# PinataFarms/DAD-3DHeads

Measured on AMD Instinct MI355X. Metric: images/sec (FLAME decode + 445-lmk projection), batch 64 @ 256^2, higher is better.
Workload: dtype f32

## Files before the change

dad-3dheads_amd/_lib.py:

```python
from __future__ import annotations

import ctypes as C
import os

_HERE = os.path.dirname(os.path.abspath(__file__))
LIB_PATH = os.environ.get("DAD3D_LIB_PATH") or os.path.join(_HERE, "libdad3d_hip.so")

OK, E_INVALID, E_HIP, E_UNSUPPORTED, E_NOMEM = range(5)
ZERO_ROTATION, TO_2D, MUTATE_PARAMS, FLIP_Z, COMPAT_CROSS_B3 = 0x1, 0x2, 0x4, 0x8, 0x10
NORMAL_ACCUMULATE = 0x1
TEX_INDEX_CORNER, TEX_INDEX_REFERENCE = 0, 1
DTYPE_F32, DTYPE_U8 = 0, 1
EVAL_SELF_EXCLUDE, EVAL_MAX_K, EVAL_MAX_HEAD, EVAL_MAX_ANCHORS = 0x1, 8, 4096, 8
HEATMAP_RAW, HEATMAP_UINT8, HEATMAP_FLOAT = 0, 1, 2
OBJ_MAX_LINE_BYTES, OBJ_FLAG_NONFINITE, OBJ_FLAG_LARGE = 71, 0x1, 0x2
JSON_MAX_NUMBER_BYTES, JSON_MAX_LITERAL_BYTES, JSON_FLAG_NONFINITE = 23, 64, 0x1
JSON_PARSE_TILE_BYTES, JSON_PARSE_RECORD_INTS = 4096, 6
(JSON_PARSE_FLAG_GRAMMAR, JSON_PARSE_FLAG_DIGITS, JSON_PARSE_FLAG_BIG_INT, JSON_PARSE_FLAG_SUBNORMAL, JSON_PARSE_FLAG_OVERFLOW,
 JSON_PARSE_FLAG_AMBIGUOUS) = 0x1, 0x2, 0x4, 0x8, 0x10, 0x20
KERNEL_AUTO, KERNEL_TWO_ROLE, KERNEL_PIPELINED, KERNEL_SPLIT_BF16, KERNEL_SPLIT_F16 = 0, 1, 2, 3, 4


class Dad3dError(RuntimeError):
    def __init__(self, status: int, message: str):
        super().__init__(f"libdad3d_hip status {status}: {message}")
        self.status = status


class UnsupportedError(Dad3dError):
    pass


class FlameModelC(C.Structure):
    _fields_ = [
        ("n_verts", C.c_int32),
        ("n_betas", C.c_int32),
        ("n_joints", C.c_int32),
        ("v_template", C.c_void_p),
        ("shapedirs", C.c_void_p),
        ("posedirs", C.c_void_p),
        ("j_regressor", C.c_void_p),
        ("parents", C.c_void_p),
        ("lbs_weights", C.c_void_p),
    ]


class FlameConstsC(C.Structure):
    _fields_ = [(k, C.c_int32) for k in ("shape", "expression", "jaw", "rotation", "eyeballs", "neck", "translation", "scale")]


class LightC(C.Structure):
    _fields_ = [
        ("intensity_ambient", C.c_float),
# ... 122 lines not shown
```

dad-3dheads_amd/csrc/capi.cpp:

```cpp
#include <algorithm>
#include <cmath>
#include <cstdlib>
#include <cstring>
#include <memory>
#include <mutex>

#include "common.hpp"

namespace dad3d {

static thread_local std::string g_last_error;

void set_error(const char* fmt, ...) {
    char buf[1024];
    va_list ap;
    va_start(ap, fmt);
    vsnprintf(buf, sizeof buf, fmt, ap);
    va_end(ap);
    g_last_error = buf;
}

template <typename T>
static dad3d_status upload(T** dst, const std::vector<T>& src) {
    *dst = nullptr;
// ... 54 lines not shown
    int kernel_choice = -1;
    float* d_bwd_partials = nullptr;
    int bwd_cap = 0;
    float* d_grad_partials = nullptr;
    size_t grad_cap = 0;
    float* d_imgc = nullptr;
    unsigned* d_sync = nullptr;
    unsigned arrive_total = 0;
    int cap_nbb = 0;
    bool profiling = false;
    unsigned long long* d_trace = nullptr;
    uint64_t trace_capacity = 0;
    char* d_split_a = nullptr;
    int split_cap = 0;
    std::vector<char*> split_retired;
    hipEvent_t ev_first = nullptr, ev_last = nullptr;
    int prof_launches = 0;
    ~dad3d_flame() {
        DeviceGuard guard(device);
        for (void* p : {(void*)d_sync, (void*)d_imgc, (void*)d_bwd_partials, (void*)d_grad_partials, (void*)d_split_a}) (void)hipFree(p);
        for (char* p : split_retired) (void)hipFree(p);
        if (ev_first) (void)hipEventDestroy(ev_first);
        if (ev_last) (void)hipEventDestroy(ev_last);
    }
};

static int decode_kernel_choice() {
    static const int choice = [] {
        const char* e = getenv("DAD3D_DECODE_KERNEL");
        if (!e) return 0;
        if (e[0] == 'v' && e[1] == '1') return DAD3D_KERNEL_TWO_ROLE;
        if (std::strcmp(e, "split") == 0) return DAD3D_KERNEL_SPLIT_BF16;
        if (std::strcmp(e, "split_f16") == 0) return DAD3D_KERNEL_SPLIT_F16;
        return std::strcmp(e, "force_pipe") == 0 ? DAD3D_KERNEL_PIPELINED : DAD3D_KERNEL_AUTO;
    }();
    return choice;
}

static size_t frag_offset(int tile, int kgroups, int g, int col, int q) {
    return ((((size_t)tile * kgroups + g) * 4 + col / 16) * 64 + (col % 16) + 16 * q) * 4;
}
template <typename F>
static void for_each_fragment(std::vector<float>& pack, int n_tiles, int kgroups, F&& f) {
    for (int t = 0; t < n_tiles; ++t)
        for (int g = 0; g < kgroups; ++g)
            for (int col = 0; col < kTileCols; ++col)
                for (int q = 0; q < 4; ++q) f(t, g, col, q, &pack[frag_offset(t, kgroups, g, col, q)]);
}

static int grad_chunks(const dad3d_flame* h) { return (h->n_verts * 3 + kGradChunk - 1) / kGradChunk; }

static dad3d_status grad_inputs_prepare(dad3d_flame* h, int batch, hipStream_t s) {
    const int pad = (batch + kBlockImages - 1) / kBlockImages * kBlockImages;
    const int per_slice = grad_chunks_per_slice(pad);
    const size_t rows = (size_t)((grad_chunks(h) + per_slice - 1) / per_slice) * pad;
    bool need_pack;
    {
        std::lock_guard<std::mutex> lock(h->c->gpack_mutex);
        need_pack = h->c->d_gpack == nullptr;
    }
    const bool need_scratch = rows > h->grad_cap;
    if (!need_pack && !need_scratch) return DAD3D_OK;
    hipStreamCaptureStatus capture = hipStreamCaptureStatusNone;
    if (s != nullptr) (void)hipStreamIsCapturing(s, &capture);
    DAD3D_REQUIRE(capture == hipStreamCaptureStatusNone,
                  "the first training step of a handle (and the first at a larger batch) allocates: run it once before capturing a graph");
// ... 312 lines not shown
    if (s != nullptr) (void)hipStreamIsCapturing(s, &capture);
    DAD3D_REQUIRE(capture == hipStreamCaptureStatusNone, "the first fp16-split decode of a model builds its basis planes: run it once before capturing a graph");
    const size_t bytes = (size_t)c->n_tiles_pipe * kPipeKGroups * 4 * 64 * 4 * sizeof(float);
    float* d = nullptr;
    DAD3D_HIP_TRY(hipMalloc(reinterpret_cast<void**>(&d), bytes));
    dad3d_status st = launch_split_basis_f16(c->d_bpack_pipe, d, c->n_tiles_pipe, c->split_b_scale, s);
    if (st == DAD3D_OK && hipStreamSynchronize(s) != hipSuccess) {
        set_error("ensure_basis_f16: hipStreamSynchronize failed");
        st = DAD3D_E_HIP;
    }
    if (st) {
        (void)hipFree(d);
        return st;
    }
    c->d_bpack_f16 = d;
    return DAD3D_OK;
}

static dad3d_status ensure_split_scratch(dad3d_flame* h, int n_phase, hipStream_t s) {
    if (n_phase <= h->split_cap) return DAD3D_OK;
    hipStreamCaptureStatus capture = hipStreamCaptureStatusNone;
    if (s != nullptr) (void)hipStreamIsCapturing(s, &capture);
    DAD3D_REQUIRE(capture == hipStreamCaptureStatusNone,
                  "the first split-kernel decode of a handle (and the first at a larger batch) allocates: run it once before capturing a graph");
    if (h->d_split_a) h->split_retired.push_back(h->d_split_a);
    h->d_split_a = nullptr, h->split_cap = 0;
    DAD3D_HIP_TRY(hipMalloc(reinterpret_cast<void**>(&h->d_split_a), (size_t)n_phase * kSplitBlockBytes));
    DAD3D_HIP_TRY(hipMemsetAsync(h->d_split_a, 0, (size_t)n_phase * kSplitBlockBytes, s));
    h->split_cap = n_phase;
    return DAD3D_OK;
}

static int resolve_kernel(const dad3d_flame* h, int pinned, int batch, unsigned flags, bool posed) {
    const bool pipe_covers = h->c->d_bpack_pipe && !posed && !(flags & (DAD3D_COMPAT_CROSS_B3 | DAD3D_ZERO_ROTATION)) &&
                             (size_t)batch * h->n_verts * 12 < ((size_t)1 << 31) && (size_t)batch * std::max(h->lmk->n, 1) * 8 < ((size_t)1 << 31);
    if (pinned == DAD3D_KERNEL_TWO_ROLE || (pinned == DAD3D_KERNEL_AUTO && !pipe_covers)) return DAD3D_KERNEL_TWO_ROLE;
    if (pipe_covers) return pinned == DAD3D_KERNEL_AUTO ? DAD3D_KERNEL_PIPELINED : pinned;
    set_error("dad3d_flame_decode: the %s kernel does not cover this launch (model, flags or output size)",
              pinned == DAD3D_KERNEL_PIPELINED ? "pipelined" : "split");
    return -1;
}

static dad3d_status decode_impl(dad3d_flame* h, float* params, int batch, unsigned flags, float* verts3d, float* proj,
                                float* lmk_xy, int32_t* lmk_px, float* posed, void* stream) {
    DAD3D_REQUIRE(h, "dad3d_flame_decode: null handle");
    DAD3D_REQUIRE(batch >= 0, "dad3d_flame_decode: negative batch");
    if (batch == 0) return DAD3D_OK;
    DAD3D_REQUIRE(params, "dad3d_flame_decode: null params");
    DAD3D_REQUIRE(!((flags & DAD3D_FLIP_Z) && (flags & DAD3D_TO_2D)), "DAD3D_FLIP_Z needs a 3-component projection");
    DAD3D_REQUIRE(!(posed && (flags & DAD3D_COMPAT_CROSS_B3)), "DAD3D_COMPAT_CROSS_B3 is inference-only (dad3d_flame_decode_posed refuses it)");
    DeviceGuard guard(h->device);
    hipStream_t s = static_cast<hipStream_t>(stream);
    const int pinned = h->kernel_choice >= 0 ? h->kernel_choice : decode_kernel_choice();
    const int kernel = resolve_kernel(h, pinned, batch, flags, posed != nullptr);
    if (kernel < 0) return DAD3D_E_UNSUPPORTED;
    const LandmarkList& L = *h->lmk;
    const int n_lmk = (lmk_xy || lmk_px) ? L.n : 0;

    const bool on_sub = L.sub && !verts3d && !proj && n_lmk && !h->d_trace && pinned != DAD3D_KERNEL_PIPELINED;
    FlameConsts* c = on_sub ? L.sub.get() : h->c.get();
    const float4* vtab = on_sub ? L.d_sub_vtab : L.d_vtab;
    const int n_verts = on_sub ? L.sub_verts : h->n_verts;

    dad3d_status st;
    if (kernel == DAD3D_KERNEL_SPLIT_BF16 || kernel == DAD3D_KERNEL_SPLIT_F16) {
        DAD3D_REQUIRE(!h->d_trace, "dad3d_flame_decode: the split kernels have no trace stamps");
// ... 17 lines not shown
        sa.n_params = h->lay.n_params;
        sa.batch = batch;
        sa.n_phase = n_phase;
        sa.n_tiles = c->n_tiles_pipe;
        split_chunking(sa.n_tiles, n_phase, &sa.n_chunks, &sa.phases_per_chunk);
        sa.n_verts = n_verts;
        sa.n_lmk = n_lmk;
        sa.image_size = h->image_size;
        sa.flags = flags & 0xFFu;
        st = launch_flame_decode_split(sa, kernel, s);
    } else if (kernel == DAD3D_KERNEL_PIPELINED) {
        DAD3D_REQUIRE(!h->d_trace || h->trace_capacity >= trace_entries_pipe(h), "dad3d_flame_decode: the trace buffer holds %llu entries, "
                      "this launch stamps %llu (dad3d_flame_debug_trace_entries)", (unsigned long long)h->trace_capacity,
                      (unsigned long long)trace_entries_pipe(h));
        PipeArgs pa{};
        pa.params = params;
        pa.bpack = c->d_bpack_pipe;
        pa.vtab = vtab;
        pa.lmk_next = L.d_next;
        pa.verts3d = verts3d;
        pa.proj = proj;
        pa.lmk_xy = lmk_xy;
        pa.lmk_px = lmk_px;
        pa.trace = h->d_trace;
        pa.n_params = h->lay.n_params;
        pa.batch = batch;
        pa.n_half = (batch + kPipeHalf - 1) / kPipeHalf;
        pa.n_tiles = c->n_tiles_pipe;
        pa.n_verts = n_verts;
        pa.n_lmk = n_lmk;
        pa.image_size = h->image_size;
        pa.flags = flags & 0xFFu;
        pa.n_chunks = 1;
        if (!h->d_trace && (!proj || (flags & DAD3D_TO_2D))) pipe_chunking(pa.n_tiles, pa.n_half, &pa.chunk_half, &pa.n_chunks, &pa.wg_per_xcd);
        st = launch_flame_decode_pipe(pa, s);
    } else {
        DAD3D_REQUIRE(!h->d_trace || h->trace_capacity >= trace_entries_two_role(h, batch), "dad3d_flame_decode: the trace buffer holds %llu "
                      "entries, this launch stamps %llu (dad3d_flame_debug_trace_entries)", (unsigned long long)h->trace_capacity,
                      (unsigned long long)trace_entries_two_role(h, batch));
        if (posed && batch <= DAD3D_GRAD_INPUTS_MAX_BATCH && h->n_betas + 36 <= kGradRows && (st = grad_inputs_prepare(h, batch, s))) return st;
        const int nbb = (batch + kBlockImages - 1) / kBlockImages;
        if (nbb > h->cap_nbb) {
            DAD3D_HIP_TRY(hipDeviceSynchronize());
            if ((st = flame_reserve(h, nbb))) return st;
        }
        DecodeArgs da{};
        da.params = params;
        da.bpack = h->c->d_bpack;
        da.jdirs = h->c->d_jdirs;
        da.j0 = h->c->d_j0;
        da.weights8 = h->c->d_w8;
        da.lmk_head = L.d_head;
        da.lmk_next = L.d_next;
        da.imgc = h->d_imgc;
        da.sync = h->d_sync;
        da.verts3d = verts3d;
        da.proj = proj;
        da.lmk_xy = lmk_xy;
        da.lmk_px = lmk_px;
        da.posed = posed;
        da.trace = h->d_trace;
        da.lay = h->lay;
        std::copy(h->parents, h->parents + kNumJoints, da.parents);
        da.batch = batch;
        da.nbb = nbb;
        da.n_tiles = h->n_tiles;
// ... 51 lines not shown
    float* d_p = n_p ? d_par + n_par + n_v : nullptr;
    float* d_lx = n_lx ? d_par + n_par + n_v + n_p : nullptr;
    int32_t* d_lp = n_lp ? reinterpret_cast<int32_t*>(d_par + n_par + n_v + n_p + n_lx) : nullptr;
    dad3d_status st = DAD3D_OK;
    auto fail = [&](hipError_t e, const char* what) {
        if (e != hipSuccess && st == DAD3D_OK) {
            set_error("%s failed: %s", what, hipGetErrorString(e));
            st = DAD3D_E_HIP;
        }
    };
    fail(hipMemcpy(d_par, params, n_par * sizeof(float), hipMemcpyHostToDevice), "hipMemcpy(params)");
    if (!st) st = dad3d_flame_decode(h, d_par, batch, flags, d_v, d_p, d_lx, d_lp, nullptr);
    if (!st) fail(hipDeviceSynchronize(), "hipDeviceSynchronize");
    if (!st && (flags & DAD3D_MUTATE_PARAMS)) fail(hipMemcpy(params, d_par, n_par * sizeof(float), hipMemcpyDeviceToHost), "hipMemcpy");
    if (!st && n_v) fail(hipMemcpy(verts3d, d_v, n_v * sizeof(float), hipMemcpyDeviceToHost), "hipMemcpy");
    if (!st && n_p) fail(hipMemcpy(proj, d_p, n_p * sizeof(float), hipMemcpyDeviceToHost), "hipMemcpy");
    if (!st && n_lx) fail(hipMemcpy(lmk_xy, d_lx, n_lx * sizeof(float), hipMemcpyDeviceToHost), "hipMemcpy");
    if (!st && n_lp) fail(hipMemcpy(lmk_px, d_lp, n_lp * sizeof(int32_t), hipMemcpyDeviceToHost), "hipMemcpy");
    (void)hipFree(d);
    return st;
}

dad3d_status dad3d_flame_readjust_params(dad3d_flame* h, float* params, int batch, const float* pads_scale,
                                         float pad_left, float pad_top, float scale, void* stream) {
    DAD3D_REQUIRE(h && batch >= 0, "dad3d_flame_readjust_params: bad argument");
    if (batch == 0) return DAD3D_OK;
    DAD3D_REQUIRE(params, "dad3d_flame_readjust_params: null params");
    DeviceGuard guard(h->device);
    return launch_readjust(params, batch, h->lay, pads_scale, pad_left, pad_top, scale, h->image_size,
                           static_cast<hipStream_t>(stream));
}

dad3d_status dad3d_flame_select_kernel(dad3d_flame* h, int which) {
    DAD3D_REQUIRE(h && which >= DAD3D_KERNEL_AUTO && which <= DAD3D_KERNEL_SPLIT_F16, "dad3d_flame_select_kernel: bad argument");
    h->kernel_choice = which;
    return DAD3D_OK;
}

dad3d_status dad3d_flame_handoff_timeouts(dad3d_flame* h, unsigned* count) {
    DAD3D_REQUIRE(h && count, "null argument");
    DeviceGuard guard(h->device);
    DAD3D_HIP_TRY(hipDeviceSynchronize());
    DAD3D_HIP_TRY(hipMemcpy(count, h->d_sync + 1, sizeof(unsigned), hipMemcpyDeviceToHost));
    return DAD3D_OK;
}

uint64_t dad3d_flame_debug_trace_entries(const dad3d_flame* h, int batch) {
    if (!h || batch <= 0) return 0;
    return std::max(trace_entries_two_role(h, batch), trace_entries_pipe(h));
}

dad3d_status dad3d_flame_debug_trace(dad3d_flame* h, unsigned long long* device_buffer, uint64_t capacity) {
    DAD3D_REQUIRE(h, "null handle");
    h->d_trace = device_buffer;
    h->trace_capacity = device_buffer ? capacity : 0;
    return DAD3D_OK;
}

dad3d_status dad3d_flame_decode_backward(dad3d_flame* h, int batch, unsigned flags, const float* consts, const float* posed,
                                         const float* grad_verts3d, const float* grad_proj, float* grad_posed,
                                         float* grad_consts, void* stream) {
    DAD3D_REQUIRE(h, "dad3d_flame_decode_backward: null handle");
    DAD3D_REQUIRE(batch >= 0, "dad3d_flame_decode_backward: negative batch");
    if (batch == 0) return DAD3D_OK;
    DAD3D_REQUIRE(consts && posed && grad_posed && grad_consts, "dad3d_flame_decode_backward: null argument");
    DAD3D_REQUIRE(grad_verts3d || grad_proj, "dad3d_flame_decode_backward: no upstream gradient");
    DAD3D_REQUIRE(!((flags & DAD3D_FLIP_Z) && (flags & DAD3D_TO_2D)), "DAD3D_FLIP_Z needs a 3-component projection");
// ... 1117 lines not shown
```

dad-3dheads_amd/csrc/common.hpp:

```cpp
#pragma once

#include <hip/hip_runtime.h>

#include <atomic>
#include <cstdarg>
#include <cstdint>
#include <cstdio>
#include <string>
#include <vector>

#include "../../include/dad3d.h"

namespace dad3d {

void set_error(const char* fmt, ...);

#define DAD3D_HIP_TRY(expr)                                                                      \
    do {                                                                                         \
        hipError_t e__ = (expr);                                                                 \
        if (e__ != hipSuccess) {                                                                 \
            ::dad3d::set_error("%s failed: %s (%s:%d)", #expr, hipGetErrorString(e__), __FILE__, \
                               __LINE__);                                                        \
            return DAD3D_E_HIP;                                                                  \
        }                                                                                        \
// ... 69 lines not shown
    ParamLayout lay;
    int parents[kNumJoints];
    int batch, nbb, n_tiles, n_tiles_pad8, n_verts, n_lmk;
    int n_pose_blocks, n_pose_blocks_pad8;
    int n_betas, max_shape;
    int betas_contiguous;
    int kgroups;
    unsigned arrive_target;
    unsigned spin_limit;
    float image_size;
    unsigned flags;
    float* posed;
};

dad3d_status launch_flame_decode(const DecodeArgs& a, hipStream_t s);

constexpr int kPipeTileVerts = 20;
constexpr int kPipeHalf = 32;
constexpr int kPipeKGroups = 26;
struct PipeArgs {
    float* params;
    const float* bpack;
    const float4* vtab;
    const int* lmk_next;
    float* verts3d;
    float* proj;
    float* lmk_xy;
    int32_t* lmk_px;
    unsigned long long* trace;
    int n_params, batch, n_half, n_tiles, n_verts, n_lmk;
    float image_size;
    unsigned flags;
    int chunk_half, n_chunks, wg_per_xcd;
};
inline void pipe_chunking(int n_tiles, int n_half, int* chunk_half, int* n_chunks, int* wg_per_xcd) {
    *chunk_half = 0, *n_chunks = 1, *wg_per_xcd = 0;
    const int max_chunks = 256 / n_tiles;
    if (max_chunks < 2 || n_half < 2) return;
    *chunk_half = (n_half + max_chunks - 1) / max_chunks;
    *n_chunks = (n_half + *chunk_half - 1) / *chunk_half;
    *wg_per_xcd = (n_tiles * *n_chunks + 7) / 8;
}
dad3d_status launch_flame_decode_pipe(const PipeArgs& a, hipStream_t s);
size_t flame_decode_pipe_lds_bytes();

constexpr int kSplitRows = 16;
constexpr int kSplitKGroups = 13;
constexpr int kSplitRowBytes = 848;
constexpr int kSplitPlaneBytes = (3 * kSplitRows * kSplitRowBytes + 1023) / 1024 * 1024;
constexpr int kSplitConstBytes = (kSplitRows * 24 * 4 + 1023) / 1024 * 1024;
constexpr int kSplitBlockBytes = kSplitPlaneBytes + kSplitConstBytes;
struct SplitArgs {
    float* params;
    const float* bpack;
    const float* bpack_f16;
    const float4* vtab;
    const int* lmk_next;
    float* verts3d;
    float* proj;
    float* lmk_xy;
    int32_t* lmk_px;
    char* aplanes;
    float b_scale;
    int n_params, batch, n_phase, n_tiles, n_verts, n_lmk;
    int n_chunks, phases_per_chunk;
    float image_size;
// ... 320 lines not shown
```

dad-3dheads_amd/csrc/flame_decode_pipe.hip:

```cpp
#pragma clang fp contract(off)
#include "common.hpp"
#include "flame_math.hpp"
#include "flame_pipe_epilogue.hpp"

#ifndef DAD3D_PIPE_STAGER_PRIO
#define DAD3D_PIPE_STAGER_PRIO 0
#endif

namespace dad3d {

namespace {

using namespace pipe;

constexpr int KG = kPipeKGroups;
constexpr int HB = kPipeHalf;
constexpr int TV = kPipeTileVerts;
constexpr int kNumBeta = 400;
constexpr int kJawCol = 3 * TV;
constexpr int LD = 424;
constexpr int OS = 76;
constexpr int CS = 24;
constexpr int kRound = 128;
struct Lds {
// ... 23 lines not shown
                                            Hook&& hook) {
    float4 an[RB] = {};
    if (G0 == 0) {
        if (FIRST) wait_ge(parts, 4);
#pragma unroll
        for (int m = 0; m < RB; ++m) af[m] = *reinterpret_cast<const float4*>(afrag + m * 16 * LD);
    }
#pragma unroll
    for (int G = G0; G < G1; ++G) {
        if (FIRST && G + 1 == 8) wait_ge(parts + 1, 4);
        if (FIRST && G + 1 == 16) wait_ge(parts + 2, 4 + RB / 2);
        if (G + 1 < KG) {
#pragma unroll
            for (int m = 0; m < RB; ++m) an[m] = *reinterpret_cast<const float4*>(afrag + m * 16 * LD + 16 * (G + 1));
        }
        __builtin_amdgcn_sched_barrier(0);
#pragma unroll
        for (int s = 0; s < 4; ++s) {
            const float bv = s == 0 ? bq[G].x : s == 1 ? bq[G].y : s == 2 ? bq[G].z : bq[G].w;
#pragma unroll
            for (int m = 0; m < RB; ++m) {
                const float av = s == 0 ? af[m].x : s == 1 ? af[m].y : s == 2 ? af[m].z : af[m].w;
                acc[m] = __builtin_amdgcn_mfma_f32_16x16x4f32(av, bv, acc[m], 0, 0, 0);
            }
        }
        __builtin_amdgcn_sched_barrier(0);
#pragma unroll
        for (int m = 0; m < RB; ++m) af[m] = an[m];
        hook(G);
        __builtin_amdgcn_sched_barrier(0);
    }
}

}

template <bool TO2D, bool CHUNKED>
__global__ __launch_bounds__(512, 2) void flame_decode_pipe_kernel(PipeArgs a) {
    extern __shared__ __attribute__((aligned(16))) float smem[];
    float* abuf = smem + Lds::a_off;
    float* otile = smem + Lds::o_off;
    float* cst = smem + Lds::c_off;
    lds_int* parts = (lds_int*)(smem + Lds::y_off);

    const int tid = threadIdx.x, lane = tid & 63, wave = tid >> 6;
    int tile_id = blockIdx.x;
    if (CHUNKED) {
        const int w = (blockIdx.x & 7) * a.wg_per_xcd + (blockIdx.x >> 3);
        if ((int)(blockIdx.x >> 3) >= a.wg_per_xcd || w >= a.n_tiles * a.n_chunks) return;
        tile_id = w / a.n_chunks;
        const int b0 = (w % a.n_chunks) * a.chunk_half * HB;
        a.params += (size_t)b0 * a.n_params;
        if (a.verts3d) a.verts3d += (size_t)b0 * a.n_verts * 3;
        if (a.proj) a.proj += (size_t)b0 * a.n_verts * (TO2D ? 2 : 3);
        if (a.lmk_xy) a.lmk_xy += (size_t)b0 * a.n_lmk * 2;
        if (a.lmk_px) a.lmk_px += (size_t)b0 * a.n_lmk * 2;
        a.batch = min(a.batch - b0, a.chunk_half * HB);
        a.n_half = (a.batch + HB - 1) / HB;
    }
    const int tile = tile_id, v0 = tile * TV;
    const int H = a.n_half, B = a.batch, P = a.n_params;
    unsigned long long* trace = a.trace ? a.trace + ((size_t)tile * 8 + wave) * 32 : nullptr;
    auto stamp = [&](int slot) {
        if (trace && lane == 0) trace[slot] = __builtin_readcyclecounter();
    };
    if (trace && lane == 0) trace[12] = wall_clock64();
    stamp(0);
    if (tid < 4) __hip_atomic_store(parts + tid, 0, __ATOMIC_RELAXED, __HIP_MEMORY_SCOPE_WORKGROUP);
    const unsigned nl = (unsigned)a.n_lmk;
    EpiCtx cx;
    const __amdgpu_buffer_rsrc_t rs3 = __builtin_amdgcn_make_buffer_rsrc(reinterpret_cast<char*>(a.verts3d), 0, 0x7fffffff, 0x00020000);
    const __amdgpu_buffer_rsrc_t rsp = __builtin_amdgcn_make_buffer_rsrc(reinterpret_cast<char*>(a.proj), 0, 0x7fffffff, 0x00020000);
    cx.lx = reinterpret_cast<char*>(a.lmk_xy), cx.lp = reinterpret_cast<char*>(a.lmk_px);
    cx.lmk_next = a.lmk_next;
    cx.image_size = a.image_size;
    cx.zsign = (a.flags & DAD3D_FLIP_Z) ? -1.0f : 1.0f;
    float4* const vt_lds = reinterpret_cast<float4*>(smem + Lds::v_off);
    auto final_epilogue = [&](int hb) {
        const int fi = lane & 3, fu = lane >> 2, fli = 4 * wave + fi, b = hb * HB + fli;
        const float4* cp = reinterpret_cast<const float4*>(cst + (((hb >> 2) & 1) * kRound + (hb & 3) * HB + fli) * CS);
        const float4 c0 = cp[0], c1 = cp[1], c2 = cp[2], c3 = cp[3], c4 = cp[4], c5 = cp[5];
        const float* ot = otile + (hb & 1) * (HB * OS) + fli * OS;
        const float jx = ot[kJawCol], jy = ot[kJawCol + 1], jz = ot[kJawCol + 2];
        const unsigned vrow = (unsigned)b * (unsigned)a.n_verts + (unsigned)(v0 + fu), bnl = (unsigned)b * nl;
        {
            const float4 t = vt_lds[fu];
            const bool live = b < B && v0 + fu < a.n_verts;
            finish_vertex<TO2D, 0>(cx, rs3, rsp, c0, c1, c2, c3, c4, c5, jx, jy, jz, ot[3 * fu], ot[3 * fu + 1], ot[3 * fu + 2], t.x, t.y, __float_as_int(t.z), __float_as_int(t.w),
                                   live && a.verts3d != nullptr, live && a.proj != nullptr, live && nl > 0 && __float_as_int(t.z) >= 0, vrow, bnl);
        }
        if (fu < TV - 16) {
            const int j = fu + 16;
            const float4 t = vt_lds[j];
            const bool live = b < B && v0 + j < a.n_verts;
            finish_vertex<TO2D, 16>(cx, rs3, rsp, c0, c1, c2, c3, c4, c5, jx, jy, jz, ot[3 * j], ot[3 * j + 1], ot[3 * j + 2], t.x, t.y, __float_as_int(t.z), __float_as_int(t.w),
                                    live && a.verts3d != nullptr, live && a.proj != nullptr, live && nl > 0 && __float_as_int(t.z) >= 0, vrow, bnl);
        }
    };

    if (wave >= 4) {
        if (DAD3D_PIPE_STAGER_PRIO) __builtin_amdgcn_s_setprio(DAD3D_PIPE_STAGER_PRIO);
        const int fw = wave - 4;
        const int lr = lane >> 5, lc = lane & 31;
        float4 pre[13];
        float4 pre1[13];
        auto load_rows = [&](int hb, float4 (&dst)[13]) {
            const int r0 = hb * HB + 8 * fw;
            const float* prow[4];
#pragma unroll
            for (int jj = 0; jj < 4; ++jj) prow[jj] = a.params + (size_t)min(r0 + 2 * jj + lr, B - 1) * P + 4 * lc;
#pragma unroll
            for (int sl = 0; sl < 3; ++sl)
#pragma unroll
                for (int jj = 0; jj < 4; ++jj) {
                    const f4u v = *reinterpret_cast<const f4u*>(prow[jj] + 128 * sl);
                    dst[4 * sl + jj] = float4{v.x, v.y, v.z, v.w};
                    __builtin_amdgcn_sched_barrier(0);
                }
            const f4u v = *reinterpret_cast<const f4u*>(a.params + (size_t)min(r0 + (lc >> 2), B - 1) * P + 384 + 4 * (lane & 3));
            dst[12] = float4{v.x, v.y, v.z, v.w};
        };
        auto write_rows = [&](int hb, int j0, int j1, const float4 (&src)[13]) {
            float* img = abuf + (hb & 1) * (HB * LD);
#pragma unroll
            for (int idx = 0; idx < 12; ++idx)
                if (idx >= j0 && idx < j1) *reinterpret_cast<float4*>(img + (8 * fw + 2 * (idx & 3) + lr) * LD + 128 * (idx >> 2) + 4 * lc) = src[idx];
            if (j1 == 13 && lane < 32) *reinterpret_cast<float4*>(img + (8 * fw + (lane >> 2)) * LD + 384 + 4 * (lane & 3)) = src[12];
        };
        auto load_a = [&](int hb) { load_rows(hb, pre); };
        auto write_a = [&](int hb, int j0, int j1) { write_rows(hb, j0, j1, pre); };
        auto write_tail = [&](int hb) {
            if (lane < 32) {
                const int r = 8 * fw + (lane >> 2), q = lane & 3;
                const float* c = cst + (((hb >> 2) & 1) * kRound + (hb & 3) * HB + r) * CS;
                float4 v = *reinterpret_cast<const float4*>(c + 4 * min(q, 2));
// ... 47 lines not shown
    auto load_raw = [&](int r) {
        const float* prow = a.params + (size_t)min(r * kRound + 32 * wave + (lane & 31), B - 1) * P + kNumBeta;
        raw0 = *reinterpret_cast<const f4u*>(prow), raw1 = *reinterpret_cast<const f4u*>(prow + 4), raw2 = *reinterpret_cast<const f3u*>(prow + 8);
        raw_scale = prow[12];
    };
    auto write_round = [&](int r, bool first) {
        const float jaw[3] = {raw0.x, raw0.y, raw0.z};
        const float rot6[6] = {raw0.w, raw1.x, raw1.y, raw1.z, raw1.w, raw2.x};
        float D[9], G[9];
        rodrigues_minus_identity_lean(jaw, D);
        rot6_to_matrix_lean(rot6, G);
        const float sp1 = raw_scale + 1.0f;
        const float s = sp1 < 1e-8f ? 1e-8f : sp1;
        if (first && wave == 0 && lane < 32) {
            float4* tail = reinterpret_cast<float4*>(abuf + lane * LD + kNumBeta);
            tail[0] = float4{D[0], D[1], D[2], D[3]};
            tail[1] = float4{D[4], D[5], D[6], D[7]};
            tail[2] = float4{D[8], 1.0f, 0.f, 0.f};
            tail[3] = float4{0.f, 0.f, 0.f, 0.f};
        }
        if (lane < 32) {
            float4* c = reinterpret_cast<float4*>(cst + ((r & 1) * kRound + 32 * wave + lane) * CS);
            c[0] = float4{D[0], D[1], D[2], D[3]};
            c[1] = float4{D[4], D[5], D[6], D[7]};
            c[2] = float4{D[8], G[0], G[1], G[2]};
            c[3] = float4{G[3], G[4], G[5], G[6]};
            c[4] = float4{G[7], G[8], s, raw2.y};
            c[5] = float4{raw2.z, 0.f, 0.f, 0.f};
            const int b = r * kRound + 32 * wave + lane;
            if ((a.flags & DAD3D_MUTATE_PARAMS) && tile == 0 && b < B)
                a.params[(size_t)b * P + kNumBeta + 11] = 0.0f;
        }
    };
    load_raw(0);
    float4 bq[KG];
    const int ei = lane & 7, eu = lane >> 3, li = 8 * wave + ei;
    float vW[3], vw2[3];
    int lh[3], ln[3];
    bool vl[3];
#pragma unroll
    for (int k = 0; k < 3; ++k) vl[k] = eu + 8 * k < TV && v0 + eu + 8 * k < a.n_verts;
    float4 k0, k1, k2, k3, k4, k5;
    auto load_consts = [&](int hb) {
        const float4* c = reinterpret_cast<const float4*>(cst + (((hb >> 2) & 1) * kRound + (hb & 3) * HB + li) * CS);
        k0 = c[0], k1 = c[1], k2 = c[2], k3 = c[3], k4 = c[4], k5 = c[5];
    };
    float jx = 0.f, jy = 0.f, jz = 0.f, ex = 0.f, ey = 0.f, ez = 0.f;
    const float* ot_e = nullptr;
    unsigned e_vrow = 0, e_bnl = 0;
    bool live3[3] = {false, false, false}, livep[3] = {false, false, false}, livel[3] = {false, false, false};
    auto epi_begin = [&](int hb) {
        ot_e = otile + (hb & 1) * (HB * OS) + li * OS;
        jx = ot_e[kJawCol], jy = ot_e[kJawCol + 1], jz = ot_e[kJawCol + 2];
        const int b = hb * HB + li;
        e_vrow = (unsigned)b * (unsigned)a.n_verts + (unsigned)(v0 + eu);
        e_bnl = (unsigned)b * nl;
#pragma unroll
        for (int k = 0; k < 3; ++k) {
            const bool live = b < B && vl[k];
            live3[k] = live && a.verts3d != nullptr, livep[k] = live && a.proj != nullptr, livel[k] = live && nl > 0 && lh[k] >= 0;
        }
    };
    auto epi_fetch = [&](int k) {
        const int j = eu + 8 * k;
        ex = ot_e[3 * j], ey = ot_e[3 * j + 1], ez = ot_e[3 * j + 2];
    };
    auto epi_finish = [&](int k) {
        if (k == 0) finish_vertex<TO2D, 0>(cx, rs3, rsp, k0, k1, k2, k3, k4, k5, jx, jy, jz, ex, ey, ez, vW[0], vw2[0], lh[0], ln[0], live3[0], livep[0], livel[0], e_vrow, e_bnl);
        if (k == 1) finish_vertex<TO2D, 8>(cx, rs3, rsp, k0, k1, k2, k3, k4, k5, jx, jy, jz, ex, ey, ez, vW[1], vw2[1], lh[1], ln[1], live3[1], livep[1], livel[1], e_vrow, e_bnl);
        if (k == 2) finish_vertex<TO2D, 16>(cx, rs3, rsp, k0, k1, k2, k3, k4, k5, jx, jy, jz, ex, ey, ez, vW[2], vw2[2], lh[2], ln[2], live3[2], livep[2], livel[2], e_vrow, e_bnl);
    };
    int hook_hb = 0;
    auto epi_hook = [&](int G) {
        if (DAD3D_PIPE_ABLATE & 2) return;
        if (G == 0) epi_begin(hook_hb), epi_fetch(0);
        if (G == 3) epi_finish(0), epi_fetch(1);
        if (G == 11) epi_finish(1), epi_fetch(2);
        if (G == 19) epi_finish(2);
    };
    auto no_hook = [](int) {};
    const float* afrag0 = abuf + (lane & 15) * LD + 4 * (lane >> 4);
    float* const ot0 = otile + ((lane >> 4) * 4) * OS + wave * 16 + (lane & 15);
    auto park = [&](int h, const f32x4 (&acc)[2]) {
        float* ot = ot0 + (h & 1) * (HB * OS);
#pragma unroll
        for (int m = 0; m < 2; ++m)
#pragma unroll
            for (int q = 0; q < 4; ++q) ot[(m * 16 + q) * OS] = acc[m][q];
    };
    const int n_rounds = (B + kRound - 1) / kRound;

    stamp(6);
    phase_barrier();
    stamp(7);
#pragma unroll
    for (int G = 0; G < KG; ++G) {
        bq[G] = bsrc[(size_t)G * 256];
        __builtin_amdgcn_sched_barrier(0);
    }
#pragma unroll
    for (int k = 0; k < 3; ++k) {
        const float4 t = a.vtab[min(v0 + eu + 8 * k, a.n_verts - 1)];
        vW[k] = t.x, vw2[k] = t.y, lh[k] = __float_as_int(t.z), ln[k] = __float_as_int(t.w);
    }
    {
        f32x4 acc[2] = {f32x4{0.f, 0.f, 0.f, 0.f}, f32x4{0.f, 0.f, 0.f, 0.f}};
        float4 af[2];
        stamp(16);
        gemm_groups<true, 0, 7, 2>(afrag0, bq, acc, af, parts, no_hook);
        stamp(1);
        write_round(0, true);
        if (wave == 0) arrive(parts + 2, lane);
        stamp(4);
        phase_barrier();
        gemm_groups<true, 7, KG, 2>(afrag0, bq, acc, af, parts, no_hook);
        stamp(2);
        park(0, acc);
        stamp(17);
    }
    if (H > 1) load_consts(0);
    phase_barrier();
    stamp(18);
#pragma unroll 1
    for (int h = 1; h < H; ++h) {
        const int r = (h + 2) >> 2;
        if (!(DAD3D_PIPE_ABLATE & 4) && (h & 3) == 2 && r < n_rounds) write_round(r, false);
        if ((h & 3) == 1 && ((h + 3) >> 2) < n_rounds) load_raw((h + 3) >> 2);
        if (h < 4) stamp(16 + 4 * h);
        f32x4 acc[2] = {f32x4{0.f, 0.f, 0.f, 0.f}, f32x4{0.f, 0.f, 0.f, 0.f}};
        float4 af[2];
        hook_hb = h - 1;
        gemm_groups<false, 0, KG, 2>(afrag0 + (h & 1) * (HB * LD), bq, acc, af, parts, epi_hook);
        park(h, acc);
        if (h < 4) stamp(17 + 4 * h);
        if (h + 1 < H) load_consts(h);
        phase_barrier();
        if (h < 4) stamp(18 + 4 * h);
    }
    stamp(3);
    final_epilogue(H - 1);
    stamp(5);
    if (trace && lane == 0) trace[13] = wall_clock64();
}

size_t flame_decode_pipe_lds_bytes() { return (size_t)Lds::total * sizeof(float); }

dad3d_status launch_flame_decode_pipe(const PipeArgs& a, hipStream_t s) {
    static PerDeviceOnce attr_done;
    const int dev = PerDeviceOnce::current();
    const size_t lds = flame_decode_pipe_lds_bytes();
    if (!attr_done.done(dev)) {
        for (const void* k : {reinterpret_cast<const void*>(&flame_decode_pipe_kernel<true, false>),
                              reinterpret_cast<const void*>(&flame_decode_pipe_kernel<false, false>),
                              reinterpret_cast<const void*>(&flame_decode_pipe_kernel<true, true>)})
            DAD3D_HIP_TRY(hipFuncSetAttribute(k, hipFuncAttributeMaxDynamicSharedMemorySize, (int)lds));
        attr_done.set(dev);
    }
    const bool to2d = (a.flags & DAD3D_TO_2D) || !a.proj;
    if (a.chunk_half > 0 && to2d) {
        hipLaunchKernelGGL((flame_decode_pipe_kernel<true, true>), dim3(8 * a.wg_per_xcd), dim3(512), lds, s, a);
    } else if (to2d) hipLaunchKernelGGL((flame_decode_pipe_kernel<true, false>), dim3(a.n_tiles), dim3(512), lds, s, a);
    else hipLaunchKernelGGL((flame_decode_pipe_kernel<false, false>), dim3(a.n_tiles), dim3(512), lds, s, a);
    DAD3D_HIP_TRY(hipGetLastError());
    return DAD3D_OK;
}

}
```

dad-3dheads_amd/flame.py:

```python
from __future__ import annotations

import ctypes as C
import io
import os
import pickle
from dataclasses import dataclass
from types import SimpleNamespace
from typing import Any, Dict, Optional, Sequence

import numpy as np
import torch
from torch import Tensor

from . import _lib
from .synthetic import load_static

FLAME_CONSTS: Dict[str, int] = {
    "shape": 300,
    "expression": 100,
    "rotation": 6,
    "jaw": 3,
    "eyeballs": 0,
    "neck": 0,
    "translation": 3,
# ... 116 lines not shown
        )
        consts_c = _lib.FlameConstsC(**{k: int(consts[k]) for k in _SLICE_ORDER})
        handle = C.c_void_p()
        _lib.check(lib.dad3d_flame_create(C.byref(model_c), C.byref(consts_c), float(image_size), self.device_index, C.byref(handle)))
        self._handle = handle
        self._lib = lib
        self.n_params = lib.dad3d_flame_num_params(handle)
        self.n_landmarks = 0
        self.landmark_indices = np.zeros((0,), dtype=np.int64)

    def __del__(self):
        h = self.__dict__.get("_handle")
        self.__dict__["_handle"] = None
        if h:
            try:
                self._lib.dad3d_flame_destroy(h)
            except Exception:
                pass

    @property
    def torch_device(self) -> torch.device:
        return torch.device("cuda", self.device_index)

    def fork(self) -> "FLAMELayer":
        handle = C.c_void_p()
        _lib.check(self._lib.dad3d_flame_fork(self._handle, C.byref(handle)))
        twin = object.__new__(type(self))
        twin.__dict__ = {k: (dict(v) if isinstance(v, dict) else v) for k, v in self.__dict__.items()}
        twin.__dict__["_handle"] = handle
        return twin

    def select_kernel(self, which: str = "auto") -> None:
        code = {"auto": _lib.KERNEL_AUTO, "two_role": _lib.KERNEL_TWO_ROLE, "pipelined": _lib.KERNEL_PIPELINED,
                "split_bf16": _lib.KERNEL_SPLIT_BF16, "split_f16": _lib.KERNEL_SPLIT_F16}[which]
        _lib.check(self._lib.dad3d_flame_select_kernel(self._handle, code))

    def decode_tables(self):
        t = self.__dict__.get("_decode_tables")
        if t is None:
            from .autograd import DecodeTables

            t = DecodeTables.from_layer(self)
            self.__dict__["_decode_tables"] = t
        return t

    def set_landmarks(self, indices: Sequence[int]) -> None:
        idx = np.ascontiguousarray(np.asarray(indices, dtype=np.int64))
        _lib.check(self._lib.dad3d_flame_set_landmarks(self._handle, idx.ctypes.data, int(idx.size)))
        self.n_landmarks = int(idx.size)
        self.landmark_indices = idx

    def decode(self, params: Tensor, *, verts3d: bool = False, proj: bool = False, to_2d: bool = True,
               landmarks: bool = False, landmarks_px: bool = False, zero_rot: bool = False, flip_z: bool = False,
               mutate: bool = False, out: Optional[Dict[str, Tensor]] = None) -> Dict[str, Tensor]:
        if params.ndim != 2:
            raise AssertionError("tensor_3dmm.ndim == 2 expected")
        if params.shape[1] != self.n_params:
            raise ValueError(f"expected {self.n_params} params per row, got {params.shape[1]}")
        if params.requires_grad and torch.is_grad_enabled():
            raise RuntimeError("FLAMELayer.decode is the raw launch (no grad_fn); differentiate through "
                               "HeadMesh.vertices_3d / reprojected_vertices or autograd.decode_with_grad")
        if params.device != self.torch_device or params.dtype != torch.float32 or not params.is_contiguous():
            raise ValueError("params must be a contiguous float32 tensor on " + str(self.torch_device))
        b, v = params.shape[0], self.n_verts
        res: Dict[str, Tensor] = {} if out is None else out
        dev = params.device

# ... 40 lines not shown
```

include/dad3d.h:

```cpp
#ifndef DAD3D_H_
#define DAD3D_H_

#include <stddef.h>
#include <stdint.h>

#ifndef DAD3D_EXPORT
#define DAD3D_EXPORT __attribute__((visibility("default")))
#endif

#ifdef __cplusplus
extern "C" {
#endif

#define DAD3D_VERSION 100

typedef enum dad3d_status {
    DAD3D_OK = 0,
    DAD3D_E_INVALID = 1,
    DAD3D_E_HIP = 2,
    DAD3D_E_UNSUPPORTED = 3,
    DAD3D_E_NOMEM = 4
} dad3d_status;

DAD3D_EXPORT const char* dad3d_last_error(void);
// ... 41 lines not shown

DAD3D_EXPORT dad3d_status dad3d_flame_decode(dad3d_flame* h, float* params, int batch, unsigned flags, float* verts3d, float* proj,
                                float* lmk_xy, int32_t* lmk_px, void* stream);

DAD3D_EXPORT dad3d_status dad3d_flame_decode_posed(dad3d_flame* h, float* params, int batch, unsigned flags, float* verts3d, float* proj,
                                      float* posed, void* stream);

DAD3D_EXPORT dad3d_status dad3d_flame_decode_backward(dad3d_flame* h, int batch, unsigned flags, const float* consts, const float* posed,
                                         const float* grad_verts3d, const float* grad_proj, float* grad_posed,
                                         float* grad_consts, void* stream);

#define DAD3D_GRAD_INPUTS_MAX_BATCH 96
DAD3D_EXPORT dad3d_status dad3d_flame_grad_inputs(dad3d_flame* h, const float* grad_posed, int batch, float* grad_inputs, void* stream);

DAD3D_EXPORT int dad3d_flame_num_chain_inputs(const dad3d_flame* h);
DAD3D_EXPORT dad3d_status dad3d_flame_pose_chain(dad3d_flame* h, const float* params, int batch, float* inputs, float* consts, void* stream);
DAD3D_EXPORT dad3d_status dad3d_flame_pose_chain_backward(dad3d_flame* h, const float* params, int batch, const float* grad_inputs,
                                             const float* grad_consts, float* grad_params, void* stream);

DAD3D_EXPORT dad3d_status dad3d_flame_decode_host(dad3d_flame* h, float* params, int batch, unsigned flags, float* verts3d,
                                     float* proj, float* lmk_xy, int32_t* lmk_px);

DAD3D_EXPORT dad3d_status dad3d_flame_readjust_params(dad3d_flame* h, float* params, int batch, const float* pads_scale,
                                         float pad_left, float pad_top, float scale, void* stream);

DAD3D_EXPORT dad3d_status dad3d_flame_profile_begin(dad3d_flame* h, void* stream);
DAD3D_EXPORT dad3d_status dad3d_flame_profile_end(dad3d_flame* h, void* stream, double* total_ms, int* launches);
DAD3D_EXPORT dad3d_status dad3d_flame_handoff_timeouts(dad3d_flame* h, unsigned* count);
#define DAD3D_KERNEL_AUTO 0
#define DAD3D_KERNEL_TWO_ROLE 1
#define DAD3D_KERNEL_PIPELINED 2
#define DAD3D_KERNEL_SPLIT_BF16 3
#define DAD3D_KERNEL_SPLIT_F16 4
DAD3D_EXPORT dad3d_status dad3d_flame_select_kernel(dad3d_flame* h, int which);
DAD3D_EXPORT dad3d_status dad3d_flame_debug_trace(dad3d_flame* h, unsigned long long* device_buffer, uint64_t capacity);
DAD3D_EXPORT uint64_t dad3d_flame_debug_trace_entries(const dad3d_flame* h, int batch);


typedef struct dad3d_mesh dad3d_mesh;

DAD3D_EXPORT dad3d_status dad3d_mesh_create(const int32_t* triangles, int ntri, int nver, int device, dad3d_mesh** out);
DAD3D_EXPORT void dad3d_mesh_destroy(dad3d_mesh* m);

#define DAD3D_NORMAL_ACCUMULATE 0x1u
DAD3D_EXPORT dad3d_status dad3d_mesh_get_normal(dad3d_mesh* m, float* ver_normal, const float* vertices, int batch,
                                   unsigned flags, void* stream);
DAD3D_EXPORT dad3d_status dad3d_mesh_get_tri_normal(dad3d_mesh* m, float* tri_normal, const float* vertices, int batch,
                                       int norm_flg, void* stream);
DAD3D_EXPORT dad3d_status dad3d_mesh_get_ver_normal(dad3d_mesh* m, float* ver_normal, const float* tri_normal, int batch,
                                       unsigned flags, void* stream);

DAD3D_EXPORT dad3d_status dad3d_mesh_rasterize(dad3d_mesh* m, uint8_t* image, const float* vertices, const float* colors,
                                  float* depth, int batch, int h, int w, int c, float alpha, int reverse,
                                  void* stream);
DAD3D_EXPORT dad3d_status dad3d_mesh_rasterize_triangles(dad3d_mesh* m, const float* vertices, float* depth,
                                            int32_t* triangle_buffer, float* barycentric, int batch, int h, int w,
                                            void* stream);

typedef struct dad3d_light {
    float intensity_ambient, intensity_directional, intensity_specular, specular_exp;
    float color_ambient[3], color_directional[3], light_pos[3], view_pos[3];
} dad3d_light;
DAD3D_EXPORT dad3d_status dad3d_mesh_phong_light(dad3d_mesh* m, float* light, const float* vertices, const float* normals,
                                    int batch, const dad3d_light* cfg, void* stream);
DAD3D_EXPORT dad3d_status dad3d_mesh_normal_phong_light(dad3d_mesh* m, float* light, float* ver_normal, const float* vertices,
                                           int batch, const dad3d_light* cfg, void* stream);
// ... 140 lines not shown
```

Measured before the change: 4.999 million.

## Add short-batch specialized pipelined FLAME decode schedule for one-to-two half batches

Adds a SHORT template variant of the pipelined decode kernel, used for un-chunked launches when the batch is between one and two pipe halves. In that variant the stager waves prefetch parameter slabs and compute the pose constants ahead of time. The compute waves run the first 48 rows as one GEMM pass, then handle the remaining 16 rows in a row-block GEMM whose hooks interleave the epilogue of earlier rows. This is meant to cut round-loop overhead and idle time between stages for the batch-64 case. It adds code complexity and a new kernel instantiation, and the previous schedule can still be forced through a 'pipelined_steady' selector.

```diff
diff --git a/dad-3dheads_amd/_lib.py b/dad-3dheads_amd/_lib.py
--- a/dad-3dheads_amd/_lib.py
+++ b/dad-3dheads_amd/_lib.py
@@ -18,7 +18,7 @@
 JSON_PARSE_TILE_BYTES, JSON_PARSE_RECORD_INTS = 4096, 6
 (JSON_PARSE_FLAG_GRAMMAR, JSON_PARSE_FLAG_DIGITS, JSON_PARSE_FLAG_BIG_INT, JSON_PARSE_FLAG_SUBNORMAL, JSON_PARSE_FLAG_OVERFLOW,
  JSON_PARSE_FLAG_AMBIGUOUS) = 0x1, 0x2, 0x4, 0x8, 0x10, 0x20
-KERNEL_AUTO, KERNEL_TWO_ROLE, KERNEL_PIPELINED, KERNEL_SPLIT_BF16, KERNEL_SPLIT_F16 = 0, 1, 2, 3, 4
+KERNEL_AUTO, KERNEL_TWO_ROLE, KERNEL_PIPELINED, KERNEL_SPLIT_BF16, KERNEL_SPLIT_F16, KERNEL_PIPELINED_STEADY = 0, 1, 2, 3, 4, 5
 
 
 class Dad3dError(RuntimeError):
diff --git a/dad-3dheads_amd/csrc/capi.cpp b/dad-3dheads_amd/csrc/capi.cpp
--- a/dad-3dheads_amd/csrc/capi.cpp
+++ b/dad-3dheads_amd/csrc/capi.cpp
@@ -110,6 +110,7 @@
         if (e[0] == 'v' && e[1] == '1') return DAD3D_KERNEL_TWO_ROLE;
         if (std::strcmp(e, "split") == 0) return DAD3D_KERNEL_SPLIT_BF16;
         if (std::strcmp(e, "split_f16") == 0) return DAD3D_KERNEL_SPLIT_F16;
+        if (std::strcmp(e, "pipe_steady") == 0) return DAD3D_KERNEL_PIPELINED_STEADY;
         return std::strcmp(e, "force_pipe") == 0 ? DAD3D_KERNEL_PIPELINED : DAD3D_KERNEL_AUTO;
     }();
     return choice;
@@ -488,6 +489,7 @@
 }
 
 static int resolve_kernel(const dad3d_flame* h, int pinned, int batch, unsigned flags, bool posed) {
+    if (pinned == DAD3D_KERNEL_PIPELINED_STEADY) pinned = DAD3D_KERNEL_AUTO;
     const bool pipe_covers = h->c->d_bpack_pipe && !posed && !(flags & (DAD3D_COMPAT_CROSS_B3 | DAD3D_ZERO_ROTATION)) &&
                              (size_t)batch * h->n_verts * 12 < ((size_t)1 << 31) && (size_t)batch * std::max(h->lmk->n, 1) * 8 < ((size_t)1 << 31);
     if (pinned == DAD3D_KERNEL_TWO_ROLE || (pinned == DAD3D_KERNEL_AUTO && !pipe_covers)) return DAD3D_KERNEL_TWO_ROLE;
@@ -571,6 +573,7 @@
         pa.image_size = h->image_size;
         pa.flags = flags & 0xFFu;
         pa.n_chunks = 1;
+        pa.short_ok = pinned != DAD3D_KERNEL_PIPELINED_STEADY;
         if (!h->d_trace && (!proj || (flags & DAD3D_TO_2D))) pipe_chunking(pa.n_tiles, pa.n_half, &pa.chunk_half, &pa.n_chunks, &pa.wg_per_xcd);
         st = launch_flame_decode_pipe(pa, s);
     } else {
@@ -688,7 +691,7 @@
 }
 
 dad3d_status dad3d_flame_select_kernel(dad3d_flame* h, int which) {
-    DAD3D_REQUIRE(h && which >= DAD3D_KERNEL_AUTO && which <= DAD3D_KERNEL_SPLIT_F16, "dad3d_flame_select_kernel: bad argument");
+    DAD3D_REQUIRE(h && which >= DAD3D_KERNEL_AUTO && which <= DAD3D_KERNEL_PIPELINED_STEADY, "dad3d_flame_select_kernel: bad argument");
     h->kernel_choice = which;
     return DAD3D_OK;
 }
diff --git a/dad-3dheads_amd/csrc/common.hpp b/dad-3dheads_amd/csrc/common.hpp
--- a/dad-3dheads_amd/csrc/common.hpp
+++ b/dad-3dheads_amd/csrc/common.hpp
@@ -125,6 +125,7 @@
     float image_size;
     unsigned flags;
     int chunk_half, n_chunks, wg_per_xcd;
+    int short_ok;
 };
 inline void pipe_chunking(int n_tiles, int n_half, int* chunk_half, int* n_chunks, int* wg_per_xcd) {
     *chunk_half = 0, *n_chunks = 1, *wg_per_xcd = 0;
diff --git a/dad-3dheads_amd/csrc/flame_decode_pipe.hip b/dad-3dheads_amd/csrc/flame_decode_pipe.hip
--- a/dad-3dheads_amd/csrc/flame_decode_pipe.hip
+++ b/dad-3dheads_amd/csrc/flame_decode_pipe.hip
@@ -79,10 +79,27 @@
     }
 }
 
-}
-
-template <bool TO2D, bool CHUNKED>
+template <int G, class Hook>
+__device__ __forceinline__ void gemm_row_block(const float* afrag, const float4 (&bq)[KG], f32x4& acc, float4& f0, float4& f1, Hook&& hook) {
+    float4 f2 = {};
+    if (G + 2 < KG) f2 = *reinterpret_cast<const float4*>(afrag + 16 * (G + 2));
+    __builtin_amdgcn_sched_barrier(0);
+    acc = __builtin_amdgcn_mfma_f32_16x16x4f32(f0.x, bq[G].x, acc, 0, 0, 0);
+    acc = __builtin_amdgcn_mfma_f32_16x16x4f32(f0.y, bq[G].y, acc, 0, 0, 0);
+    acc = __builtin_amdgcn_mfma_f32_16x16x4f32(f0.z, bq[G].z, acc, 0, 0, 0);
+    acc = __builtin_amdgcn_mfma_f32_16x16x4f32(f0.w, bq[G].w, acc, 0, 0, 0);
+    __builtin_amdgcn_sched_barrier(0);
+    f0 = f1, f1 = f2;
+    hook(std::integral_constant<int, G>{});
+    __builtin_amdgcn_sched_barrier(0);
+    if constexpr (G + 1 < KG) gemm_row_block<G + 1>(afrag, bq, acc, f0, f1, hook);
+}
+
+}
+
+template <bool TO2D, bool CHUNKED, bool SHORT = false>
 __global__ __launch_bounds__(512, 2) void flame_decode_pipe_kernel(PipeArgs a) {
+    static_assert(!(SHORT && CHUNKED), "the short schedule is for un-chunked launches");
     extern __shared__ __attribute__((aligned(16))) float smem[];
     float* abuf = smem + Lds::a_off;
     float* otile = smem + Lds::o_off;
@@ -144,9 +161,118 @@
         }
     };
 
+    auto final_rows16 = [&]() {
+        const int fu = min(lane & 31, TV - 1), fli = 3 * 16 + 2 * wave + (lane >> 5), b = fli;
+        const float4* cp = reinterpret_cast<const float4*>(cst + fli * CS);
+        const float4 c0 = cp[0], c1 = cp[1], c2 = cp[2], c3 = cp[3], c4 = cp[4], c5 = cp[5];
+        const float* ot = otile + fli * OS;
+        const float jx = ot[kJawCol], jy = ot[kJawCol + 1], jz = ot[kJawCol + 2];
+        const unsigned vrow = (unsigned)b * (unsigned)a.n_verts + (unsigned)(v0 + fu), bnl = (unsigned)b * nl;
+        const float4 t = vt_lds[fu];
+        const bool live = b < B && (lane & 31) < TV && v0 + fu < a.n_verts;
+        finish_vertex<TO2D, 0>(cx, rs3, rsp, c0, c1, c2, c3, c4, c5, jx, jy, jz, ot[3 * fu], ot[3 * fu + 1], ot[3 * fu + 2], t.x, t.y, __float_as_int(t.z), __float_as_int(t.w),
+                               live && a.verts3d != nullptr, live && a.proj != nullptr, live && nl > 0 && __float_as_int(t.z) >= 0, vrow, bnl);
+    };
+    const bool two_pass = B > 48;
+
     if (wave >= 4) {
         if (DAD3D_PIPE_STAGER_PRIO) __builtin_amdgcn_s_setprio(DAD3D_PIPE_STAGER_PRIO);
         const int fw = wave - 4;
+        if constexpr (SHORT) {
+            const int lr = lane >> 5, lc = lane & 31;
+            float4 pre[4][3][2], pre_t;
+            auto load_slab = [&](int rb, int sl) {
+#pragma unroll
+                for (int jj = 0; jj < 2; ++jj) {
+                    const f4u v = *reinterpret_cast<const f4u*>(a.params + (size_t)min(16 * rb + 4 * fw + 2 * jj + lr, B - 1) * P + 128 * sl + 4 * lc);
+                    pre[rb][sl][jj] = float4{v.x, v.y, v.z, v.w};
+                    __builtin_amdgcn_sched_barrier(0);
+                }
+            };
+            auto write_slab = [&](int rb, int sl) {
+#pragma unroll
+                for (int jj = 0; jj < 2; ++jj) *reinterpret_cast<float4*>(abuf + (16 * rb + 4 * fw + 2 * jj + lr) * LD + 128 * sl + 4 * lc) = pre[rb][sl][jj];
+            };
+#pragma unroll
+            for (int rb = 0; rb < 3; ++rb) load_slab(rb, 0);
+            const float* ptail = a.params + (size_t)min(16 * fw + (lane & 15), B - 1) * P + kNumBeta;
+            const f4u raw0 = *reinterpret_cast<const f4u*>(ptail), raw1 = *reinterpret_cast<const f4u*>(ptail + 4);
+            const f3u raw2 = *reinterpret_cast<const f3u*>(ptail + 8);
+            const float raw_scale = ptail[12];
+            const float4 vt_row = a.vtab[min(v0 + min(lane, TV - 1), a.n_verts - 1)];
+            stamp(1);
+            phase_barrier();
+            stamp(6);
+#pragma unroll
+            for (int sl = 1; sl < 3; ++sl)
+#pragma unroll
+                for (int rb = 0; rb < 3; ++rb) load_slab(rb, sl);
+            {
+                const f4u v = *reinterpret_cast<const f4u*>(a.params + (size_t)min(16 * fw + (lane >> 2), B - 1) * P + 384 + 4 * (lane & 3));
+                pre_t = float4{v.x, v.y, v.z, v.w};
+            }
+#pragma unroll
+            for (int rb = 0; rb < 3; ++rb) write_slab(rb, 0);
+            arrive(parts, lane);
+            stamp(7);
+#pragma unroll
+            for (int sl = 0; sl < 3; ++sl) load_slab(3, sl);
+            {
+                const float jaw[3] = {raw0.x, raw0.y, raw0.z};
+                const float rot6[6] = {raw0.w, raw1.x, raw1.y, raw1.z, raw1.w, raw2.x};
+                float D[9], G[9];
+                rodrigues_minus_identity_lean(jaw, D);
+                rot6_to_matrix_lean(rot6, G);
+                const float sp1 = raw_scale + 1.0f;
+                const float s = sp1 < 1e-8f ? 1e-8f : sp1;
+                if (lane < 16) {
+                    const int b = 16 * fw + lane;
+                    float4* tail = reinterpret_cast<float4*>(abuf + b * LD + kNumBeta);
+                    tail[0] = float4{D[0], D[1], D[2], D[3]};
+                    tail[1] = float4{D[4], D[5], D[6], D[7]};
+                    tail[2] = float4{D[8], 1.0f, 0.f, 0.f};
+                    tail[3] = float4{0.f, 0.f, 0.f, 0.f};
+                    float4* c = reinterpret_cast<float4*>(cst + b * CS);
+                    c[0] = float4{D[0], D[1], D[2], D[3]};
+                    c[1] = float4{D[4], D[5], D[6], D[7]};
+                    c[2] = float4{D[8], G[0], G[1], G[2]};
+                    c[3] = float4{G[3], G[4], G[5], G[6]};
+                    c[4] = float4{G[7], G[8], s, raw2.y};
+                    c[5] = float4{raw2.z, 0.f, 0.f, 0.f};
+                    if ((a.flags & DAD3D_MUTATE_PARAMS) && tile == 0 && b < B)
+                        a.params[(size_t)b * P + kNumBeta + 11] = 0.0f;
+                }
+            }
+            arrive(parts + 3, lane);
+            stamp(4);
+#pragma unroll
+            for (int rb = 0; rb < 3; ++rb) write_slab(rb, 1);
+            arrive(parts + 1, lane);
+#pragma unroll
+            for (int rb = 0; rb < 3; ++rb) write_slab(rb, 2);
+            *reinterpret_cast<float4*>(abuf + (16 * fw + (lane >> 2)) * LD + 384 + 4 * (lane & 3)) = pre_t;
+            arrive(parts + 2, lane);
+            stamp(2);
+            if (fw == 3 && lane < TV) vt_lds[lane] = vt_row;
+            if (two_pass) {
+#pragma unroll
+                for (int sl = 0; sl < 3; ++sl) write_slab(3, sl);
+            }
+            stamp(17);
+            phase_barrier();
+            stamp(19);
+            if (two_pass) {
+                phase_barrier();
+                stamp(23);
+                final_rows16();
+            } else {
+                final_epilogue(0);
+                final_epilogue(1);
+            }
+            stamp(5);
+            if (trace && lane == 0) trace[13] = wall_clock64();
+            return;
+        }
         const int lr = lane >> 5, lc = lane & 31;
         float4 pre[13];
         float4 pre1[13];
@@ -260,7 +386,7 @@
                 a.params[(size_t)b * P + kNumBeta + 11] = 0.0f;
         }
     };
-    load_raw(0);
+    if constexpr (!SHORT) load_raw(0);
     float4 bq[KG];
     const int ei = lane & 7, eu = lane >> 3, li = 8 * wave + ei;
     float vW[3], vw2[3];
@@ -316,6 +442,99 @@
 #pragma unroll
             for (int q = 0; q < 4; ++q) ot[(m * 16 + q) * OS] = acc[m][q];
     };
+    if constexpr (SHORT) {
+        stamp(6);
+        phase_barrier();
+        stamp(7);
+#pragma unroll
+        for (int G = 0; G < KG; ++G) {
+            bq[G] = bsrc[(size_t)G * 256];
+            __builtin_amdgcn_sched_barrier(0);
+        }
+#pragma unroll
+        for (int k = 0; k < 3; ++k) {
+            const float4 t = a.vtab[min(v0 + eu + 8 * k, a.n_verts - 1)];
+            vW[k] = t.x, vw2[k] = t.y, lh[k] = __float_as_int(t.z), ln[k] = __float_as_int(t.w);
+        }
+        {
+            f32x4 acc[3] = {f32x4{0.f, 0.f, 0.f, 0.f}, f32x4{0.f, 0.f, 0.f, 0.f}, f32x4{0.f, 0.f, 0.f, 0.f}};
+            float4 af[3];
+            stamp(16);
+            wait_ge(parts, 4);
+            gemm_groups<false, 0, KG, 3>(afrag0, bq, acc, af, parts, [&](int G) {
+                if (G == 6) stamp(1), wait_ge(parts + 1, 4);
+                if (G == 14) wait_ge(parts + 2, 4);
+                if (G == 23) wait_ge(parts + 3, 4);
+            });
+            stamp(2);
+#pragma unroll
+            for (int m = 0; m < 3; ++m)
+#pragma unroll
+                for (int q = 0; q < 4; ++q) ot0[(m * 16 + q) * OS] = acc[m][q];
+            stamp(17);
+        }
+        if (!two_pass) {
+            phase_barrier();
+            stamp(18);
+            stamp(3);
+            final_epilogue(0);
+            final_epilogue(1);
+            stamp(5);
+            if (trace && lane == 0) trace[13] = wall_clock64();
+            return;
+        }
+        load_consts(0);
+        phase_barrier();
+        stamp(18);
+        const int fu = lane >> 2, b2 = HB + 4 * wave + (lane & 3);
+        float4 tb = {};
+        bool lv = false;
+        auto b_begin = [&]() {
+            const float4* c = reinterpret_cast<const float4*>(cst + b2 * CS);
+            k0 = c[0], k1 = c[1], k2 = c[2], k3 = c[3], k4 = c[4], k5 = c[5];
+            ot_e = otile + b2 * OS;
+            jx = ot_e[kJawCol], jy = ot_e[kJawCol + 1], jz = ot_e[kJawCol + 2];
+            e_vrow = (unsigned)b2 * (unsigned)a.n_verts + (unsigned)(v0 + fu);
+            e_bnl = (unsigned)b2 * nl;
+        };
+        auto b_fetch = [&](int j, bool in_tile) {
+            ex = ot_e[3 * j], ey = ot_e[3 * j + 1], ez = ot_e[3 * j + 2];
+            tb = vt_lds[j];
+            lv = in_tile && b2 < B && v0 + j < a.n_verts;
+        };
+        auto b_finish = [&](auto voff) {
+            finish_vertex<TO2D, decltype(voff)::value>(cx, rs3, rsp, k0, k1, k2, k3, k4, k5, jx, jy, jz, ex, ey, ez, tb.x, tb.y, __float_as_int(tb.z), __float_as_int(tb.w),
+                                                       lv && a.verts3d != nullptr, lv && a.proj != nullptr, lv && nl > 0 && __float_as_int(tb.z) >= 0, e_vrow, e_bnl);
+        };
+        auto short_hook = [&](auto group) {
+            constexpr int G = decltype(group)::value;
+            if constexpr (DAD3D_PIPE_ABLATE & 2) return;
+            if constexpr (G == 0) epi_begin(0), epi_fetch(0);
+            if constexpr (G == 3) epi_finish(0), epi_fetch(1);
+            if constexpr (G == 7) epi_finish(1), epi_fetch(2);
+            if constexpr (G == 11) epi_finish(2);
+            if constexpr (G == 12) b_begin(), b_fetch(fu, true);
+            if constexpr (G == 16) b_finish(std::integral_constant<int, 0>{}), b_fetch(min(fu + 16, TV - 1), fu + 16 < TV);
+            if constexpr (G == 20) b_finish(std::integral_constant<int, 16>{});
+        };
+        {
+            f32x4 acc = f32x4{0.f, 0.f, 0.f, 0.f};
+            const float* af3 = afrag0 + 3 * 16 * LD;
+            stamp(20);
+            float4 f0 = *reinterpret_cast<const float4*>(af3), f1 = *reinterpret_cast<const float4*>(af3 + 16);
+            gemm_row_block<0>(af3, bq, acc, f0, f1, short_hook);
+#pragma unroll
+            for (int q = 0; q < 4; ++q) ot0[(3 * 16 + q) * OS] = acc[q];
+            stamp(21);
+        }
+        phase_barrier();
+        stamp(22);
+        stamp(3);
+        final_rows16();
+        stamp(5);
+        if (trace && lane == 0) trace[13] = wall_clock64();
+        return;
+    }
     const int n_rounds = (B + kRound - 1) / kRound;
 
     stamp(6);
@@ -380,13 +599,18 @@
     if (!attr_done.done(dev)) {
         for (const void* k : {reinterpret_cast<const void*>(&flame_decode_pipe_kernel<true, false>),
                               reinterpret_cast<const void*>(&flame_decode_pipe_kernel<false, false>),
-                              reinterpret_cast<const void*>(&flame_decode_pipe_kernel<true, true>)})
+                              reinterpret_cast<const void*>(&flame_decode_pipe_kernel<true, true>),
+                              reinterpret_cast<const void*>(&flame_decode_pipe_kernel<true, false, true>),
+                              reinterpret_cast<const void*>(&flame_decode_pipe_kernel<false, false, true>)})
             DAD3D_HIP_TRY(hipFuncSetAttribute(k, hipFuncAttributeMaxDynamicSharedMemorySize, (int)lds));
         attr_done.set(dev);
     }
     const bool to2d = (a.flags & DAD3D_TO_2D) || !a.proj;
     if (a.chunk_half > 0 && to2d) {
         hipLaunchKernelGGL((flame_decode_pipe_kernel<true, true>), dim3(8 * a.wg_per_xcd), dim3(512), lds, s, a);
+    } else if (a.chunk_half == 0 && a.short_ok && a.batch > kPipeHalf && a.batch <= 2 * kPipeHalf) {
+        if (to2d) hipLaunchKernelGGL((flame_decode_pipe_kernel<true, false, true>), dim3(a.n_tiles), dim3(512), lds, s, a);
+        else hipLaunchKernelGGL((flame_decode_pipe_kernel<false, false, true>), dim3(a.n_tiles), dim3(512), lds, s, a);
     } else if (to2d) hipLaunchKernelGGL((flame_decode_pipe_kernel<true, false>), dim3(a.n_tiles), dim3(512), lds, s, a);
     else hipLaunchKernelGGL((flame_decode_pipe_kernel<false, false>), dim3(a.n_tiles), dim3(512), lds, s, a);
     DAD3D_HIP_TRY(hipGetLastError());
diff --git a/dad-3dheads_amd/flame.py b/dad-3dheads_amd/flame.py
--- a/dad-3dheads_amd/flame.py
+++ b/dad-3dheads_amd/flame.py
@@ -172,7 +172,8 @@
 
     def select_kernel(self, which: str = "auto") -> None:
         code = {"auto": _lib.KERNEL_AUTO, "two_role": _lib.KERNEL_TWO_ROLE, "pipelined": _lib.KERNEL_PIPELINED,
-                "split_bf16": _lib.KERNEL_SPLIT_BF16, "split_f16": _lib.KERNEL_SPLIT_F16}[which]
+                "split_bf16": _lib.KERNEL_SPLIT_BF16, "split_f16": _lib.KERNEL_SPLIT_F16,
+                "pipelined_steady": _lib.KERNEL_PIPELINED_STEADY}[which]
         _lib.check(self._lib.dad3d_flame_select_kernel(self._handle, code))
 
     def decode_tables(self):
diff --git a/include/dad3d.h b/include/dad3d.h
--- a/include/dad3d.h
+++ b/include/dad3d.h
@@ -97,6 +97,7 @@
 #define DAD3D_KERNEL_PIPELINED 2
 #define DAD3D_KERNEL_SPLIT_BF16 3
 #define DAD3D_KERNEL_SPLIT_F16 4
+#define DAD3D_KERNEL_PIPELINED_STEADY 5
 DAD3D_EXPORT dad3d_status dad3d_flame_select_kernel(dad3d_flame* h, int which);
 DAD3D_EXPORT dad3d_status dad3d_flame_debug_trace(dad3d_flame* h, unsigned long long* device_buffer, uint64_t capacity);
 DAD3D_EXPORT uint64_t dad3d_flame_debug_trace_entries(const dad3d_flame* h, int batch);
```

New measurement: 4.674 million. 6.5% lower.
